# bystrogenomics/bystro-vcf

Measured on AMD Instinct MI355X. Metric: variants/sec, higher is better.
Workload: dtype u8; 1 GPU; BASELINE configs[2]: 1KG-Phase3 chr1-shaped, 2504 samples, biallelic SNPs; rows_per_block=311296, resident_blocks_per_gpu=8, n_samples=2504, input=resident in HBM, blocks_in_flight=3, flags=default (--allowFilter PASS,.), class maps on

## Files before the change

bystro-vcf_amd/__init__.py:

```python
import ctypes as C
import os

import numpy as np

try:
    import torch
except ImportError:
    torch = None

_HERE = os.path.dirname(os.path.abspath(__file__))
LIB_PATH = os.environ.get("BVCF_LIB") or os.path.join(_HERE, "libbvcf.so")

if not os.path.exists(LIB_PATH):
    raise ImportError(
        "bystro-vcf_amd: %s not built (run `python -c 'import __graft_entry__ as g; g.build()'` "
        "or `make -C bystro-vcf_amd/csrc`); there is no fallback path" % LIB_PATH)

lib = C.CDLL(LIB_PATH)

ABI_VERSION = 9
ABI_VERSION_SUBSET = 10
DEVICE_PAD = 64
NO_CMAP = 0xFFFFFFFF

OK, E_ARG, E_HIP, E_NODEV, E_BUSY, E_EMPTY, E_TOO_BIG, E_CAPACITY, E_NOMEM, E_FATAL = 0, -1, -2, -3, -4, -5, -6, -7, -8, -9
LINE_OK, LINE_FIELDS, LINE_FILTER, LINE_NOALLELE = 0, 1, 2, 3
SITE_NAMES = ["SNP", "INS", "DEL", "MNP", "MULTIALLELIC"]
ALT_BASE, ALT_INS, ALT_DEL = 0, 1, 2
CLS_NONE, CLS_HET, CLS_HOM, CLS_MISSING = 0, 1, 2, 3
SAMPLE_STATS_COLUMNS = ["sample", "het", "hom", "missing", "transitions", "transversions", "heterozygosity", "homozygosity",
                        "missingness", "trTv"]

BENCH_EXPORTS = ["bvcf_bench_device", "bvcf_bench_device_slots", "bvcf_bench_stream_kernel", "bvcf_bench_head_left"]

PLAN_EXPORTS = ["bvcf_plan_text_ranges", "bvcf_plan_bgzf_ranges", "bvcf_cut_text_range", "bvcf_find_bgzf_chain",
                "bvcf_plan_threads", "bvcf_plan_fd", "bvcf_head_fast_line"]

EXPORTS = [
    "bvcf_create", "bvcf_destroy", "bvcf_last_error", "bvcf_version", "bvcf_reserve", "bvcf_set_sample_names", "bvcf_set_row_format", "bvcf_alloc_pinned", "bvcf_alloc_pinned_near", "bvcf_warmup",
    "bvcf_free_pinned", "bvcf_submit", "bvcf_submit_device", "bvcf_submit_bgzf", "bvcf_collect", "bvcf_sample_stats", "bvcf_counters", "bvcf_sum_counters",
    "bvcf_allreduce_counters", "bvcf_device_count", "bvcf_device_pci_bus_id", "bvcf_path", "bvcf_config_defaults", "bvcf_string_header", "bvcf_format_tsv", "bvcf_run_buffer", "bvcf_run_fd", "bvcf_decompress_fd", "bvcf_bgzf_inflate_device", "bvcf_bgzf_deflate_device", "bvcf_free",
    "bvcf_arrow_open", "bvcf_arrow_append", "bvcf_arrow_close",
]


class Params(C.Structure):
    _fields_ = [
        ("abi_version", C.c_uint32), ("device", C.c_int32), ("n_header_fields", C.c_uint32),
        ("eol_chars", C.c_uint32), ("eol_byte", C.c_uint8), ("want_class_maps", C.c_uint8),
        ("want_dosage", C.c_uint8), ("want_name_lists", C.c_uint8), ("allow_filter", C.c_char_p), ("exclude_filter", C.c_char_p),
        ("max_batch_bytes", C.c_uint64), ("max_lines", C.c_uint32), ("max_alleles", C.c_uint32),
        ("cmap_bytes", C.c_uint64), ("n_slots", C.c_uint32), ("path", C.c_uint32),
        ("packed_sites", C.c_uint32), ("render_sites", C.c_uint32), ("want_sample_stats", C.c_uint32),
        ("min_gq", C.c_uint32), ("min_dp", C.c_uint32), ("sample_keep", C.POINTER(C.c_uint32)),
    ]


class Config(C.Structure):
    _fields_ = [
# ... 104 lines not shown
MODE_STREAM, MODE_TEXT_RANGES, MODE_BGZF_RANGES = 0, 1, 2
BGZF_SKIP_FIRST_LINE, BGZF_END_OF_STREAM = 1, 2
lib.bvcf_plan_text_ranges.argtypes = [C.c_uint64, C.c_uint64, C.c_uint64, C.c_uint64, C.POINTER(RangePlan)]
lib.bvcf_plan_bgzf_ranges.argtypes = [C.c_uint64, C.c_uint64, C.c_uint32, C.c_uint64, C.POINTER(RangePlan)]
lib.bvcf_cut_text_range.argtypes = [C.c_char_p, C.c_uint64, C.c_uint64, C.c_int, C.c_int, C.c_uint8, C.POINTER(TextCut)]
lib.bvcf_find_bgzf_chain.argtypes = [C.c_char_p, C.c_size_t, C.c_size_t]
lib.bvcf_find_bgzf_chain.restype = C.c_long
lib.bvcf_plan_threads.argtypes = [C.c_uint32, C.c_uint32, C.c_int, C.POINTER(ThreadBudget)]
lib.bvcf_plan_fd.argtypes = [C.c_int, C.c_int, C.c_uint32, C.c_uint64, C.c_int, C.POINTER(PlanBlock), C.c_size_t,
                             C.POINTER(C.c_size_t), C.POINTER(C.c_int), C.POINTER(RangePlan)]


def plan_fd(fd_in, n_workers, max_batch_bytes=0, device_inflate=1, fd_err=2, cap=1 << 16):
    out = (PlanBlock * cap)()
    n = C.c_size_t(0)
    mode = C.c_int(-1)
    plan = RangePlan()
    rc = lib.bvcf_plan_fd(fd_in, fd_err, n_workers, max_batch_bytes, device_inflate, out, cap, C.byref(n), C.byref(mode), C.byref(plan))
    assert n.value <= cap, "more blocks than room"
    return rc, mode.value, plan, [out[i] for i in range(n.value)]


HEAD_FAST_DECLINE, HEAD_FAST_PASS, HEAD_FAST_FILTER = 0, 1, 2
HAS_HEAD_BITS, NOT_REGULAR, DEFERRED = 0x80000000, 0x40000000, 0xFFFFFFFE


def head_fast_line(head, ls, len_flags, counts, cmap_off, tab_bits, line, n_header, allow="PASS,.", exclude=""):
    lib.bvcf_head_fast_line.argtypes = [C.c_char_p, C.c_uint32, C.c_uint32, C.c_uint32, C.POINTER(C.c_uint32), C.c_uint32,
                                        C.POINTER(C.c_uint32), C.c_uint32, C.c_uint32, C.c_char_p, C.c_char_p, C.c_void_p, C.c_void_p]
    L = np.zeros(1, dtype=LINE_DTYPE)
    A = np.zeros(1, dtype=ALLELE_DTYPE)
    v = lib.bvcf_head_fast_line(bytes(head), len(head), ls, len_flags, (C.c_uint32 * 5)(*counts), cmap_off,
                                (C.c_uint32 * 8)(*tab_bits), line, n_header, allow.encode(), exclude.encode(),
                                L.ctypes.data, A.ctypes.data)
    return v, (L[0] if v != HEAD_FAST_DECLINE else None), (A[0] if v == HEAD_FAST_PASS else None)


class BvcfError(RuntimeError):
    def __init__(self, rc, msg):
        super().__init__("bvcf error %d: %s" % (rc, msg))
        self.rc = rc


def make_config(cfg=None, device=0, max_batch_bytes=0, n_format_threads=0):
    cfg = cfg or {}
    c = Config()
    lib.bvcf_config_defaults(C.byref(c))
    keep = [cfg.get("emptyField", "!").encode(), cfg.get("fieldDelimiter", ";").encode(),
            cfg.get("allow", "PASS,.").encode(), cfg.get("exclude", "").encode()]
    c.empty_field, c.field_delimiter, c.allow_filter, c.exclude_filter = keep
    c.keep_id = int(cfg.get("keepId", False))
    c.keep_info = int(cfg.get("keepInfo", False))
    c.keep_pos = int(cfg.get("keepPos", False))
    c.normalize_header = int(cfg.get("normalizeHeader", True))
    c.device = device
    c.max_batch_bytes = max_batch_bytes
    c.n_format_threads = n_format_threads
    if cfg.get("sample"):
        keep.append(cfg["sample"].encode())
# ... 404 lines not shown
```

bystro-vcf_amd/csrc/bvcf_common.hip.h:

```cpp
#pragma once

#include <hip/hip_runtime.h>
#include <stdint.h>

#include "../../include/bvcf.h"

namespace bvcf_dev {


constexpr int kWave = 64;
constexpr int kWavesPerWg = 4;
constexpr int kWgThreads = kWave * kWavesPerWg;
constexpr uint32_t kChunk = 1024;
constexpr uint32_t kMaxProducerWaves = 32768;
constexpr uint32_t kScanGroup = 1024;

typedef uint32_t u32x4 __attribute__((ext_vector_type(4)));
typedef u32x4 u32x4_u __attribute__((aligned(1)));

struct FilterTable {
  uint32_t allow_nil, allow_n;
  uint32_t deny_nil, deny_n;
  uint16_t allow_off[32], allow_len[32];
  uint16_t deny_off[32], deny_len[32];
// ... 70 lines not shown
  uint32_t fused;
  uint32_t gen_stream;
  uint32_t wide;
  uint32_t win_bytes;
  uint32_t win_tabs_cap;
  uint32_t *win_tabs;
  uint32_t tile_bytes;
  uint32_t tile_quota;
  uint32_t n_tiles;
  StreamEntry *entries;
  uint32_t *line_len;
  uint32_t *line_cmap;
  uint16_t *head_bits;
  uint32_t *line_bits;
  uint32_t *finish_items;
  uint32_t *real_tasks;
  uint32_t *left_lines;
  uint32_t head_fast;
  uint32_t s1_fmode;
  uint32_t s1_fkey[4], s1_flen[4];
};
constexpr uint32_t kHasHeadBits = 0x80000000u;
constexpr uint32_t kNotRegular = 0x40000000u;


__device__ __forceinline__ int lane_id() { return threadIdx.x & (kWave - 1); }

__device__ __forceinline__ uint32_t wave_incl_scan(uint32_t v) {
  v += (uint32_t)__builtin_amdgcn_update_dpp(0, (int)v, 0x111, 0xF, 0xF, true);
  v += (uint32_t)__builtin_amdgcn_update_dpp(0, (int)v, 0x112, 0xF, 0xF, true);
  v += (uint32_t)__builtin_amdgcn_update_dpp(0, (int)v, 0x114, 0xF, 0xF, true);
  v += (uint32_t)__builtin_amdgcn_update_dpp(0, (int)v, 0x118, 0xF, 0xF, true);
  v += (uint32_t)__builtin_amdgcn_update_dpp(0, (int)v, 0x142, 0xA, 0xF, false);
  v += (uint32_t)__builtin_amdgcn_update_dpp(0, (int)v, 0x143, 0xC, 0xF, false);
  return v;
}

__device__ __forceinline__ uint32_t wave_incl_scan_max(uint32_t v) {
  v = max(v, (uint32_t)__builtin_amdgcn_update_dpp(0, (int)v, 0x111, 0xF, 0xF, true));
  v = max(v, (uint32_t)__builtin_amdgcn_update_dpp(0, (int)v, 0x112, 0xF, 0xF, true));
  v = max(v, (uint32_t)__builtin_amdgcn_update_dpp(0, (int)v, 0x114, 0xF, 0xF, true));
  v = max(v, (uint32_t)__builtin_amdgcn_update_dpp(0, (int)v, 0x118, 0xF, 0xF, true));
  v = max(v, (uint32_t)__builtin_amdgcn_update_dpp(0, (int)v, 0x142, 0xA, 0xF, false));
  v = max(v, (uint32_t)__builtin_amdgcn_update_dpp(0, (int)v, 0x143, 0xC, 0xF, false));
  return v;
}
// ... 82 lines not shown
```

bystro-vcf_amd/csrc/bvcf_core.hip:

```cpp
#include "bvcf_device.hip.h"
#include "../../include/bvcf_bench.h"
#include "../../include/bvcf_plan.h"
#include "bvcf_bgzf.h"
#include "bvcf_bgzf_out.h"

#include <dlfcn.h>
#include <rccl/rccl.h>
#include <stdio.h>
#include <stdlib.h>
#include <string.h>

#include <algorithm>
#include <mutex>
#include <string>
#include <thread>
#include <vector>

using namespace bvcf_dev;

namespace {

struct Slot {
  hipStream_t stream = nullptr;
  bool used_gen = false;
// ... 2042 lines not shown
  if (fill_filter(allow_filter, true, &ft.allow_nil, &ft.allow_n, ft.allow_off, ft.allow_len, ft.text, &used) ||
      fill_filter(exclude_filter, false, &ft.deny_nil, &ft.deny_n, ft.deny_off, ft.deny_len, ft.text, &used))
    return -1;
  HeadFastHostBytes hb;
  memset(&hb, 0, sizeof hb);
  memcpy(hb.b, head, std::min<size_t>(head_bytes, kHeadFastBytes + 16));
  StreamEntry en;
  en.ls = ls;
  en.len = len_flags;
  en.ac = counts[0];
  en.an = counts[1];
  en.n_het = counts[2];
  en.n_hom = counts[3];
  en.n_miss = counts[4];
  en.cmap_off = cmap_off;
  HeadFastHostOut out;
  memset(&out, 0, sizeof out);
  const int v = head_fast_eval(en, tab_bits, hb, line, n_header, &ft, out);
  if (v != kHeadFastDecline) memcpy(out_line, out.Lw, sizeof out.Lw);
  if (v == kHeadFastPass) memcpy(out_allele, out.Aw, sizeof out.Aw);
  return v;
}

int bvcf_counters(bvcf_ctx *c, uint64_t out[8]) {
  if (!c || !out) return BVCF_E_ARG;
  memcpy(out, c->totals, sizeof c->totals);
  return BVCF_OK;
}

int bvcf_sum_counters(bvcf_ctx *const *ctxs, int n, uint64_t out[8]) {
  if (!ctxs || n < 0 || !out) return BVCF_E_ARG;
  for (int k = 0; k < 8; k++) out[k] = 0;
  for (int i = 0; i < n; i++) {
    if (!ctxs[i]) return BVCF_E_ARG;
    for (int k = 0; k < 8; k++) out[k] += ctxs[i]->totals[k];
  }
  return BVCF_OK;
}

int bvcf_bgzf_inflate_device(int device, const uint8_t *comp, size_t n_comp, uint8_t *out, size_t cap, size_t *n_out) {
  if ((!comp && n_comp) || !n_out || (!out && cap)) return BVCF_E_ARG;
  *n_out = 0;
  int n_dev = 0;
  if (hipGetDeviceCount(&n_dev) != hipSuccess || device < 0 || device >= n_dev) return BVCF_E_NODEV;
  std::vector<bvcf_bgzf::Block> blocks;
  const long used = bvcf_bgzf::scan(comp, n_comp, &blocks);
// ... 259 lines not shown
```

bystro-vcf_amd/csrc/bvcf_headfast.hip.h:

```cpp
#pragma once

#include <stddef.h>

#include "bvcf_common.hip.h"

namespace bvcf_dev {

constexpr uint32_t kHeadFastBytes = 64;
constexpr uint32_t kHeadFastFilter = 16;
constexpr uint32_t kHfNoTask = 0xFFFFFFFFu;
constexpr uint32_t kHfDeferred = 0xFFFFFFFEu;

enum { kHeadFastDecline = 0, kHeadFastPass = 1, kHeadFastFilterFail = 2 };

static_assert(sizeof(bvcf_line) == 64 && sizeof(bvcf_allele) == 64, "records are written as sixteen words");
static_assert(offsetof(bvcf_line, fend) == 8 && offsetof(bvcf_line, rec_first) == 44 && offsetof(bvcf_line, n_rec) == 48 &&
                  offsetof(bvcf_line, n_fields) == 52 && offsetof(bvcf_line, gt_task) == 56 && offsetof(bvcf_line, status) == 60 &&
                  offsetof(bvcf_line, site_type) == 61,
              "bvcf_line words");
static_assert(offsetof(bvcf_allele, line) == 8 && offsetof(bvcf_allele, alt_idx) == 12 && offsetof(bvcf_allele, alt_off) == 16 &&
                  offsetof(bvcf_allele, alt_len) == 20 && offsetof(bvcf_allele, ac) == 24 && offsetof(bvcf_allele, n_miss) == 40 &&
                  offsetof(bvcf_allele, cmap_off) == 44 && offsetof(bvcf_allele, ref) == 48 && offsetof(bvcf_allele, alt_base) == 49 &&
                  offsetof(bvcf_allele, kind) == 50 && offsetof(bvcf_allele, site_type) == 51 && offsetof(bvcf_allele, trtv) == 52 &&
                  offsetof(bvcf_allele, flags) == 53 && offsetof(bvcf_allele, gt_task) == 56,
              "bvcf_allele words");

__host__ __device__ __forceinline__ bool hf_is_actg(uint32_t c) {
  const uint32_t d = c - 'A';
  return d < 20u && ((0x80045u >> (d & 31u)) & 1u);
}

__host__ __device__ __forceinline__ uint32_t hf_trtv(uint32_t ref, uint32_t alt) {
  const uint32_t x = ((ref ^ alt) >> 1) & 3u;
  return (hf_is_actg(ref) && hf_is_actg(alt)) ? (x == 3u ? 1u : 2u) : 0u;
}

__host__ __device__ __forceinline__ uint32_t hf_next_bit(unsigned long long x[4]) {
  uint32_t pos = 256u;
  bool done = false;
#pragma unroll
  for (uint32_t q = 0; q < 4; q++) {
    const bool take = !done && x[q] != 0ull;
    if (take) {
      pos = 64u * q + (uint32_t)__builtin_ctzll(x[q]);
      x[q] &= x[q] - 1ull;
    }
    done = done || take;
  }
  return pos;
}

__host__ __device__ __forceinline__ uint32_t hf_byte16(const uint32_t v[4], uint32_t k) {
  const uint32_t w = k < 8u ? (k < 4u ? v[0] : v[1]) : (k < 12u ? v[2] : v[3]);
  return (w >> (8u * (k & 3u))) & 0xFFu;
}

__host__ __device__ inline bool hf_filter_in(const uint32_t f[4], uint32_t n, const uint16_t *off, const uint16_t *len, uint32_t cnt,
                                             const uint8_t *text) {
  bool hit = false;
  for (uint32_t i = 0; i < cnt; i++) {
    const uint32_t kl = len[i];
    if (kl > kHeadFastFilter) continue;
    bool eq = kl == n;
    for (uint32_t k = 0; k < kl; k++) eq = eq && hf_byte16(f, k) == text[off[i] + k];
    hit = hit || eq;
  }
  return hit;
}

template <class H, class Out>
__host__ __device__ inline int head_fast_eval(const StreamEntry &en, const uint32_t bits[8], const H &head, uint32_t g, uint32_t n_header,
                                              const FilterTable *ft, Out &out) {
  if (!(en.len & kHasHeadBits) || (en.len & kNotRegular) || en.n_miss == kHfDeferred || n_header <= 9u) return kHeadFastDecline;
  const uint32_t ls = en.ls, len = en.len & ~(kHasHeadBits | kNotRegular), sh = ls & 3u;
  unsigned long long x[4];
#pragma unroll
  for (uint32_t q = 0; q < 4; q++) x[q] = ((unsigned long long)bits[2 * q + 1] << 32) | bits[2 * q];
  uint32_t t[9];
#pragma unroll
  for (uint32_t i = 0; i < 9; i++) t[i] = hf_next_bit(x) - sh;
  if (t[8] + sh >= 256u) return kHeadFastDecline;
  if (t[6] >= kHeadFastBytes || t[8] >= len) return kHeadFastDecline;
  if (t[3] - t[2] != 2u || t[4] - t[3] != 2u) return kHeadFastDecline;
  const uint32_t f_off = t[5] + 1u, f_len = t[6] - f_off;
  if (f_len > kHeadFastFilter) return kHeadFastDecline;
  const uint32_t ref = head.byte(t[2] + 1u), alt = head.byte(t[3] + 1u);
  uint32_t fv[4];
  head.bytes16(f_off, fv);
  if (!hf_is_actg(alt) || alt == ref) return kHeadFastDecline;
  bool pass = true;
  if (!ft->allow_nil && !hf_filter_in(fv, f_len, ft->allow_off, ft->allow_len, ft->allow_n, ft->text))
    pass = false;
  else if (!ft->deny_nil && hf_filter_in(fv, f_len, ft->deny_off, ft->deny_len, ft->deny_n, ft->text))
    pass = false;
  uint32_t Lw[16];
  Lw[0] = ls;
  Lw[1] = len;
#pragma unroll
  for (uint32_t i = 0; i < 9; i++) Lw[2 + i] = t[i];
  Lw[11] = 0;
  Lw[12] = pass ? 1u : 0u;
  Lw[13] = pass ? n_header : 0u;
  Lw[14] = g;
  Lw[15] = pass ? (uint32_t)BVCF_LINE_OK | ((uint32_t)BVCF_SITE_SNP << 8) : (uint32_t)BVCF_LINE_FILTER;
  out.line(Lw);
  if (!pass) return kHeadFastFilterFail;
  uint32_t Aw[16];
  const uint32_t cm = en.cmap_off;
  const bool sparse = cm != BVCF_NO_CMAP && (cm & 1u);
  Aw[0] = Aw[1] = 0;
  Aw[2] = g;
  Aw[3] = 0;
  Aw[4] = 0;
  Aw[5] = 1;
  Aw[6] = en.ac;
  Aw[7] = en.an;
  Aw[8] = en.n_het;
  Aw[9] = en.n_hom;
  Aw[10] = en.n_miss;
  Aw[11] = cm != BVCF_NO_CMAP ? cm & ~15u : cm;
  Aw[12] = ref | (alt << 8) | ((uint32_t)BVCF_ALT_BASE << 16) | ((uint32_t)BVCF_SITE_SNP << 24);
  Aw[13] = hf_trtv(ref, alt) | ((BVCF_ALLELE_POS_TEXT | (sparse ? BVCF_ALLELE_CMAP_SPARSE : 0u)) << 8);
  Aw[14] = g;
  Aw[15] = 0;
  out.allele(Aw);
  return kHeadFastPass;
}

struct HeadFastHostBytes {
  uint8_t b[kHeadFastBytes + 16];
  __host__ __device__ uint32_t byte(uint32_t rel) const { return b[rel]; }
  __host__ __device__ void bytes16(uint32_t rel, uint32_t out[4]) const {
#pragma unroll
    for (uint32_t q = 0; q < 4; q++)
      out[q] = (uint32_t)b[rel + 4 * q] | ((uint32_t)b[rel + 4 * q + 1] << 8) | ((uint32_t)b[rel + 4 * q + 2] << 16) |
               ((uint32_t)b[rel + 4 * q + 3] << 24);
  }
};

struct HeadFastHostOut {
  uint32_t Lw[16], Aw[16];
  void line(const uint32_t w[16]) {
    for (int i = 0; i < 16; i++) Lw[i] = w[i];
  }
  void allele(const uint32_t w[16]) {
    for (int i = 0; i < 16; i++) Aw[i] = w[i];
  }
};

}
```

bystro-vcf_amd/csrc/bvcf_stream.hip.h:

```cpp
#pragma once

#include <type_traits>

#include "bvcf_common.hip.h"
#include "bvcf_gtscan.hip.h"
#include "bvcf_headfast.hip.h"

namespace bvcf_dev {


constexpr uint32_t kNone = 0xFFFFFFFFu;
constexpr uint32_t kDeferred = 0xFFFFFFFEu;
static_assert(kDeferred == kHfDeferred, "head_fast_eval's copy");

__device__ inline uint32_t find_eol(const KernelArgs &a, uint32_t from, uint32_t limit) {
  const int lane = lane_id();
  const uint32_t last_off = (a.cap - 16u) & ~3u;
  for (uint32_t base = from & ~3u; base < limit; base += 4u * kChunk) {
    u32x4 v[4];
#pragma unroll
    for (int q = 0; q < 4; q++) v[q] = ld_stream(a.buf + min(base + q * kChunk + 16u * lane, last_off));
#pragma unroll
    for (int q = 0; q < 4; q++) {
      const uint32_t off = base + q * kChunk + 16u * lane;
// ... 26 lines not shown
  const unsigned long long be = __ballot(me != 0);
  uint32_t eol_here = kNone;
  if (be) {
    const int src = __ffsll((long long)be) - 1;
    eol_here = lane_value(off + __ffs(me) - 1, src);
    mt &= bits_until(eol_here, off);
  }
  uint32_t tot;
  const uint32_t cnt = __popc(mt);
  const uint32_t prefix = wave_excl_scan(cnt, &tot);
  if (*found_io + tot >= need) {
    const uint32_t target = need - 1 - *found_io;
    const bool mine = prefix <= target && target < prefix + cnt;
    const unsigned long long bm = __ballot(mine);
    const int src = __ffsll((long long)bm) - 1;
    const uint32_t pos = mine ? off + nth_bit(mt, target - prefix) : 0u;
    return lane_value(pos, src);
  }
  *found_io += tot;
  *eolp = eol_here;
  return kNone;
}

__device__ __forceinline__ uint32_t head_window16(const KernelArgs &a, u32x4 v, uint32_t start, uint32_t *mt_out) {
  const int lane = lane_id();
  const uint32_t need = 9;
  const uint32_t base = start & ~3u;
  if (lane == 0) v.x &= 0xFFFFFFFFu << (8u * (start & 3u));
  const uint32_t off = base + 16u * lane;
  uint32_t valid = bits_until(a.nbytes, off);
  if (lane >= 16) valid = 0;
  const uint32_t e4 = a.eol_byte * 0x01010101u;
  const uint32_t eol_any = (zero_bytes(v.x ^ e4) | zero_bytes(v.y ^ e4) | zero_bytes(v.z ^ e4) | zero_bytes(v.w ^ e4));
  if (__ballot(eol_any != 0 && lane < 16)) return kNone;
  const uint32_t mt = eq_mask16(v, '\t') & valid;
  *mt_out = mt;
  const uint32_t cnt = __popc(mt);
  uint32_t x = cnt;
  x += (uint32_t)__builtin_amdgcn_update_dpp(0, (int)x, 0x111, 0xF, 0xF, true);
  x += (uint32_t)__builtin_amdgcn_update_dpp(0, (int)x, 0x112, 0xF, 0xF, true);
  x += (uint32_t)__builtin_amdgcn_update_dpp(0, (int)x, 0x114, 0xF, 0xF, true);
  x += (uint32_t)__builtin_amdgcn_update_dpp(0, (int)x, 0x118, 0xF, 0xF, true);
  const uint32_t prefix = x - cnt;
  const bool mine = lane < 16 && prefix < need && need <= x;
  const unsigned long long bm = __ballot(mine);
  if (!bm) return kNone;
  const int src = __ffsll((long long)bm) - 1;
  const uint32_t pos = mine ? off + nth_bit(mt, need - 1 - prefix) : 0u;
  return lane_value(pos, src);
}

constexpr int kPipeChunks = 10;

#ifdef BVCF_EXP_TIMES
__device__ unsigned long long g_wave_t[2][32768];
__device__ unsigned long long g_phase_t[8][32768];
__device__ unsigned int g_wave_hw[2][32768];
#if BVCF_EXP_TIMES + 0 == 2
#define STAMP(k)
#else
#define STAMP(k)                                                   \
  {                                                                \
    const unsigned long long now_ = __builtin_readcyclecounter();  \
    ph_[k] += now_ - last_;                                        \
    last_ = now_;                                                  \
  }
#endif
#else
#define STAMP(k)
#endif
__global__ __launch_bounds__(kWgThreads) void k_stream(KernelArgs a) {
#ifdef BVCF_EXP_TIMES
// ... 33 lines not shown
  uint32_t p = kNone;
  if (tile_lo < tile_hi) {
    p = 0;
    if (r0 > 0) {
      const uint32_t q = find_eol(a, r0 - 1, r1);
      p = q == kNone ? kNone : q + 1;
    }
  }

  const uint32_t lines_bound = (uint32_t)(((unsigned long long)per_wave * T) / (4ull * ns + 8ull)) + 2u;
  const uint32_t slots_per_wave = lines_bound + lines_bound / 4u;
  cm_next = wave * slots_per_wave;
  cm_end = cm_next + slots_per_wave;
  if (maps && wave == 0 && lane == 0)
    a.counters->cmap_maps = min(n_waves, a.n_tiles) * slots_per_wave;
  auto map_slot = [&]() -> uint32_t {
    if (!maps) return BVCF_NO_CMAP;
    if (cm_next >= cm_end) {
      if (lane == 0) a.counters->pad[0] = 1;
      return BVCF_NO_CMAP;
    }
    return cmap_of(a, cm_next, true);
  };
  auto commit = [&](uint32_t ls, uint32_t cend, const GtStats &st, bool deferred, uint32_t cm_off, bool bits_ok = false,
                    uint32_t bits = 0u, uint32_t n_slots = 1u) {
    while (ls >= (tile + 1) * T) {
      if (lane == 0) a.census[tile] = n_local;
      n_listed += n_local;
      tile++;
      n_local = 0;
    }
    if (n_local >= a.tile_quota) {
      if (lane == 0) a.counters->pad[0] = 1;
      return;
    }
    if (lane == 0) {
      StreamEntry en;
      en.ls = ls;
      en.len = (cend - ls) | (bits_ok ? kHasHeadBits : 0u);
      en.ac = st.ac;
      en.an = st.an;
      en.n_het = st.n_het;
      en.n_hom = st.n_hom;
      en.n_miss = deferred ? kDeferred : st.n_miss;
      en.cmap_off = cm_off;
      a.entries[(size_t)tile * a.tile_quota + n_local] = en;
    }
    if (bits_ok && lane < 16) a.head_bits[((size_t)tile * a.tile_quota + n_local) * 16u + (uint32_t)lane] = (uint16_t)bits;
    n_local++;
    if (maps && !deferred) cm_next += n_slots;
  };
  const uint32_t amask = (ns & 255u) ? 3u : 0u;
  const uint32_t cap_off = (a.cap - 16u) & ~3u;
  auto chunk_off = [&](uint32_t s_begin, uint32_t c) -> uint32_t {
    return min((s_begin & ~amask) + c * kChunk + 16u * lane, cap_off);
  };
  auto chunk_at = [&](uint32_t s_begin, uint32_t c) -> u32x4 { return ld_stream(a.buf + chunk_off(s_begin, c)); };
  auto finish_stats = [&](const FastAcc &acc, GtStats *st) {
    wave_sum3(acc.het, acc.hom, acc.miss, ns, &st->n_het, &st->n_hom, &st->n_miss);
    st->ac = st->n_het + 2u * st->n_hom;
    st->an = 2u * (ns - st->n_miss);
  };

  while (p != kNone && p < r1) {
// ... 2 lines not shown
      tab9 = head_window(a, load16(a.buf, base + 16u * lane, a.cap), base, kWave, &found, &eolp);
      if (tab9 != kNone || eolp != kNone) break;
    }
    if (tab9 == kNone) {
      if (eolp == kNone) break;
      seen++;
      p = eolp + 1;
      continue;
    }
    uint32_t s_begin = tab9 + 1;
    GtStats st = {0, 0, 0, 0, 0};
    const unsigned long long pred = (unsigned long long)s_begin + 4ull * ns - 1ull;
    uint32_t cend = kNone;

    if (pred + a.eol_chars <= nb && pipelined) {
      auto run_pipeline = [&](auto loads_tag) {
        constexpr int kLoads = decltype(loads_tag)::value;
        constexpr uint32_t nc = kLoads;
        uint32_t pA = p, sA = s_begin, peA = (uint32_t)pred;
        u32x4 va[kPipeChunks];
        u32x4 hv = {0u, 0u, 0u, 0u};
        uint32_t mtA = 0, mtB = 0;
        bool bitsA = false;
        auto head_at = [&](uint32_t start) -> u32x4 {
          return *reinterpret_cast<const u32x4_u *>(a.buf + min((start & ~3u) + 16u * (lane & 15), cap_off));
        };
        bool hv_ok = peA + 1u < r1;
        hv = head_at(hv_ok ? peA + 1u : sA);
#pragma unroll
        for (int g = 0; g < kPipeChunks; g++) va[g] = g < kLoads ? chunk_at(sA, g) : u32x4{0u, 0u, 0u, 0u};
        for (;;) {
          STAMP(0);
          uint32_t sB = 0, peB = 0;
          bool b_ok = false;
          if (hv_ok) {
            const uint32_t t9 = head_window16(a, hv, peA + 1u, &mtB);
            if (t9 != kNone) {
              sB = t9 + 1;
              const unsigned long long pb = (unsigned long long)sB + 4ull * ns - 1ull;
              if (pb + 1ull <= nb) {
                peB = (uint32_t)pb;
                b_ok = true;
              }
            }
          }
          const bool hvc_ok = b_ok && peB + 1u < r1;
          hv = head_at(hvc_ok ? peB + 1u : sA);
          STAMP(1);
          const uint32_t cmA = bcast0(map_slot());
          uint8_t *cm = cmA != BVCF_NO_CMAP ? a.cmap + cmA : nullptr;
#ifdef BVCF_EXP_NO_SPARSE
          const bool sparse_ok = false;
#else
          const bool sparse_ok = cm != nullptr && a.cmap_stride >= 4u * kSparseWords;
#endif
          FastAcc acc = {0, 0, 0, 0, sparse_ok ? 0u : kDenseMode};
          if (cm && !sparse_ok) zero_stage(stage, nc);
          const uint32_t rA = sA & amask;
          const uint32_t w0 = __builtin_amdgcn_alignbyte(__builtin_amdgcn_readfirstlane(va[0].y),
                                                         __builtin_amdgcn_readfirstlane(va[0].x), rA);
// ... 16 lines not shown
          uint32_t enc = 0, n_slots = 1;
          const uint32_t raw_slots = (kRawAreaBytes + a.cmap_stride - 1u) / a.cmap_stride;
          auto raw_area = [&]() -> uint8_t * {
            const uint32_t reserve = (r1 - min(r1, peA)) / (4u * ns + 8u) + 2u;
            if (cm_next + 1u + raw_slots + reserve > cm_end || cmap_of(a, cm_next + raw_slots, true) == BVCF_NO_CMAP) return nullptr;
            return cm + a.cmap_stride;
          };
          if (sparse_ok && acc.n_sp < kDenseMode) {
            enc = finish_list(sparse, acc, cm, min(kListAlleles, a.cmap_stride / (4u * kSparseWords)), stage, nc, a.cmap_stride,
                              acc.n_sp > BVCF_CMAP_SPARSE_MAX ? raw_area() : nullptr);
          } else if (sparse_ok && acc.n_oth == 0u) {
            enc = 1u << 1;
          } else if (sparse_ok && acc.n_oth < kDenseMode) {
            enc = finish_dense(sparse, acc.n_oth, raw_area());
          }
          if (enc == kRawEnc) n_slots += raw_slots;
          if (__any(acc.bad != 0)) {
            s_begin = sA;
            p = pA;
            break;
          }
          finish_stats(acc, &st);
          seen++;
          commit(pA, peA, st, false, cmA == BVCF_NO_CMAP ? cmA : cmA | enc, bitsA, mtA, n_slots);
          p = peA + 1u;
          if (!b_ok) {
            s_begin = kNone;
            break;
          }
          pA = peA + 1u;
          sA = sB;
          peA = peB;
          hv_ok = hvc_ok;
          mtA = mtB;
#ifdef BVCF_EXP_NO_HEAD_BITS
          bitsA = false;
#else
          bitsA = true;
#endif
          STAMP(4);
        }
      };
      switch (n_chunks) {
        case 1: run_pipeline(std::integral_constant<int, 1>{}); break;
        case 2: run_pipeline(std::integral_constant<int, 2>{}); break;
        case 3: run_pipeline(std::integral_constant<int, 3>{}); break;
        case 4: run_pipeline(std::integral_constant<int, 4>{}); break;
        case 5: run_pipeline(std::integral_constant<int, 5>{}); break;
        case 6: run_pipeline(std::integral_constant<int, 6>{}); break;
        case 7: run_pipeline(std::integral_constant<int, 7>{}); break;
        case 8: run_pipeline(std::integral_constant<int, 8>{}); break;
        case 9: run_pipeline(std::integral_constant<int, 9>{}); break;
        default: run_pipeline(std::integral_constant<int, 10>{}); break;
      }
      static_assert(kPipeChunks == 10, "the dispatch above covers 1..10 chunks");
      if (s_begin == kNone) continue;
    } else if (pred + a.eol_chars <= nb) {
      const uint32_t pe = (uint32_t)pred;
      bool term = true;
      if (a.eol_chars == 2) term = a.buf[pe + 1] == a.eol_byte && a.buf[pe] != a.eol_byte;
      if (term) {
// ... 26 lines not shown
    }
  }
  for (; tile < tile_hi; tile++) {
    if (lane == 0) a.census[tile] = n_local;
    n_listed += n_local;
    n_local = 0;
  }
  if (lane == 0) a.run_lines[wave] = n_listed;
  if (lane == 0 && seen) atomicAdd(&a.counters->lines_seen, seen);
  if (lane == 0 && n_other) atomicAdd(&a.counters->n_other_shape, n_other);
#ifdef BVCF_EXP_TIMES
  if (lane == 0) {
    g_wave_t[1][wave] = wall_clock64();
    for (int k = 0; k < 8; k++) g_phase_t[k][wave] = ph_[k];
  }
#endif
}

}
#include "bvcf_streamgen.hip.h"
namespace bvcf_dev {

struct HeadFastDeviceBytes {
  const uint8_t *p;
  uint32_t room;
  __device__ __forceinline__ uint32_t byte(uint32_t rel) const { return rel < room ? p[rel] : 0u; }
  __device__ __forceinline__ void bytes16(uint32_t rel, uint32_t out[4]) const {
    const u32x4 v = load16(p, rel, room);
    out[0] = v.x;
    out[1] = v.y;
    out[2] = v.z;
    out[3] = v.w;
  }
};

struct HeadFastDeviceOut {
  u32x4 *lp, *ap;
  __device__ __forceinline__ static void put(u32x4 *d, const uint32_t w[16]) {
#pragma unroll
    for (uint32_t q = 0; q < 4; q++) d[q] = u32x4{w[4 * q], w[4 * q + 1], w[4 * q + 2], w[4 * q + 3]};
  }
  __device__ __forceinline__ void line(const uint32_t w[16]) { put(lp, w); }
  __device__ __forceinline__ void allele(const uint32_t w[16]) { put(ap, w); }
};

__global__ __launch_bounds__(kWgThreads) void k_order(KernelArgs a) {
  __shared__ uint32_t s_part[2][kWavesPerWg];
  __shared__ uint32_t s_first[kWgThreads + 1];
  const int lane = lane_id();
  const uint32_t w = threadIdx.x >> 6;
  if (a.n_tiles == 0) {
    if (blockIdx.x == 0 && threadIdx.x == 0) a.counters->n_lines = 0;
    return;
  }
  const uint32_t pw = a.prod_waves;
  const uint32_t q_tiles = a.n_tiles / pw, r_tiles = a.n_tiles % pw;
  auto run_first = [&](uint32_t wv) -> uint32_t { return wv * q_tiles + min(wv, r_tiles); };
  const uint32_t per_wg = (pw + gridDim.x - 1u) / gridDim.x;
  const uint32_t w_lo = min(blockIdx.x * per_wg, pw), w_hi = min(w_lo + per_wg, pw);
  const uint32_t t_lo = run_first(w_lo), t_hi = run_first(w_hi);
  uint32_t sum = 0;
  {
    const uint32_t n4 = w_lo / 4u;
    const u32x4 *c4 = reinterpret_cast<const u32x4 *>(a.run_lines);
    for (uint32_t i = threadIdx.x; i < n4; i += kWgThreads) {
// ... 25 lines not shown
    for (uint32_t i = 0; i < kWavesPerWg; i++) {
      if (i < w) wbase += s_part[1][i];
      total += s_part[1][i];
    }
    s_first[threadIdx.x] = wbase + pre;
    if (threadIdx.x == 0) s_first[kWgThreads] = total;
    __syncthreads();
    const uint32_t n_round = s_first[kWgThreads];
    for (uint32_t j0 = 0; j0 < n_round; j0 += kWgThreads) {
      const uint32_t j = j0 + threadIdx.x;
      const uint32_t g = base + j;
      const bool live = j < n_round && g < a.max_lines;
      bool left = false;
      if (live) {
        uint32_t lo = 0;
#pragma unroll
        for (uint32_t s = kWgThreads / 2u; s >= 1u; s >>= 1)
          if (s_first[lo + s] <= j) lo += s;
        const uint32_t tl = lo, k = j - s_first[lo];
        const size_t ei = (size_t)(c0 + tl) * a.tile_quota + k;
        const u32x4 *ep = reinterpret_cast<const u32x4 *>(a.entries + ei);
        const u32x4 *bp = reinterpret_cast<const u32x4 *>(a.head_bits + ei * 16u);
        const u32x4 e0 = ep[0], e1 = ep[1];
        const u32x4 b0 = bp[0], b1 = bp[1];
        StreamEntry en;
        en.ls = e0.x;
        en.len = e0.y;
        en.ac = e0.z;
        en.an = e0.w;
        en.n_het = e1.x;
        en.n_hom = e1.y;
        en.n_miss = e1.z;
        en.cmap_off = e1.w;
        if (g < a.max_tasks) {
          GtResult r;
          r.ac = en.ac;
          r.an = en.an;
          r.n_het = en.n_het;
          r.n_hom = en.n_hom;
          r.n_miss = en.n_miss;
          r.n_fields = en.n_miss == kDeferred ? kDeferred : a.n_header - 9u;
          r.regular = (en.n_miss == kDeferred || (en.len & kNotRegular)) ? 0u : 1u;
          r.pad = 0;
          a.results[g] = r;
        }
        int verdict = kHeadFastDecline;
        if (a.head_fast && (en.len & kHasHeadBits) && g < a.max_alleles && g < a.max_tasks) {
          const uint32_t bits[8] = {b0.x, b0.y, b0.z, b0.w, b1.x, b1.y, b1.z, b1.w};
          const HeadFastDeviceBytes head = {a.buf + en.ls, a.cap - min(a.cap, en.ls)};
          HeadFastDeviceOut out = {reinterpret_cast<u32x4 *>(a.lines + g), reinterpret_cast<u32x4 *>(a.alleles + g)};
          verdict = head_fast_eval(en, bits, head, g, a.n_header, a.filters, out);
          if (verdict == kHeadFastFilterFail) a.alleles[g].gt_task = kHfNoTask;
        }
        if (verdict == kHeadFastDecline) {
          left = true;
          a.line_off[g] = en.ls;
          a.line_len[g] = en.len & ~kNotRegular;
          a.line_cmap[g] = en.cmap_off;
          if (en.len & kHasHeadBits) {
            u32x4 *dst = reinterpret_cast<u32x4 *>(a.line_bits + (size_t)g * 8u);
            dst[0] = bp[0];
            dst[1] = bp[1];
          }
        }
      }
      const unsigned long long lm = __ballot(left);
      if (lm) {
        uint32_t at = 0;
        if (lane == 0) at = atomicAdd(&a.counters->n_left, (uint32_t)__popcll(lm));
        at = bcast0(at) + __builtin_amdgcn_mbcnt_hi((uint32_t)(lm >> 32), __builtin_amdgcn_mbcnt_lo((uint32_t)lm, 0u));
        if (left) a.left_lines[at] = g;
      }
    }
    base += s_first[kWgThreads];
  }
  if (t_hi == a.n_tiles && threadIdx.x == 0) a.counters->n_lines = base;
}


}
// ... 1 lines not shown
```

include/bvcf_plan.h:

```cpp
#ifndef BVCF_PLAN_H
#define BVCF_PLAN_H

#include <stddef.h>
#include <stdint.h>

#include "bvcf.h"

#ifdef __cplusplus
extern "C" {
#endif

typedef struct {
  uint64_t data_off;
  uint64_t range_bytes;
  uint64_t spare_bytes;
  uint64_t n_ranges;
} bvcf_range_plan;

int bvcf_plan_text_ranges(uint64_t file_size, uint64_t data_off, uint64_t max_batch_bytes, uint64_t first_line_bytes,
                          bvcf_range_plan *out);
int bvcf_plan_bgzf_ranges(uint64_t file_size, uint64_t data_off, uint32_t n_workers, uint64_t max_batch_bytes,
                          bvcf_range_plan *out);

enum {
// ... 21 lines not shown
int bvcf_plan_threads(uint32_t cpus, uint32_t n_workers, int mode, bvcf_thread_budget *out);

typedef struct {
  uint32_t worker;
  uint32_t piece;
  uint64_t range;
  uint64_t file_off;
  uint64_t nbytes;
  uint64_t own;
  uint32_t first_off;
  uint8_t bgzf;
  uint8_t bgzf_flags;
  uint8_t last_piece;
  uint8_t reserved;
} bvcf_plan_block;

int bvcf_plan_fd(int fd_in, int fd_err, uint32_t n_workers, uint64_t max_batch_bytes, int device_inflate,
                 bvcf_plan_block *out, size_t cap, size_t *n_out, int *mode_out, bvcf_range_plan *plan_out);

int bvcf_head_fast_line(const uint8_t *head, uint32_t head_bytes, uint32_t ls, uint32_t len_flags, const uint32_t counts[5],
                        uint32_t cmap_off, const uint32_t tab_bits[8], uint32_t line, uint32_t n_header, const char *allow_filter,
                        const char *exclude_filter, bvcf_line *out_line, bvcf_allele *out_allele);

#ifdef __cplusplus
}
#endif
#endif
```

Baseline: 515.5 million variants/s.

## Encode tab positions in stream entries to skip head-bit buffer for plain lines

```diff
diff --git a/bystro-vcf_amd/__init__.py b/bystro-vcf_amd/__init__.py
--- a/bystro-vcf_amd/__init__.py
+++ b/bystro-vcf_amd/__init__.py
@@ -34,7 +34,7 @@
 BENCH_EXPORTS = ["bvcf_bench_device", "bvcf_bench_device_slots", "bvcf_bench_stream_kernel", "bvcf_bench_head_left"]
 
 PLAN_EXPORTS = ["bvcf_plan_text_ranges", "bvcf_plan_bgzf_ranges", "bvcf_cut_text_range", "bvcf_find_bgzf_chain",
-                "bvcf_plan_threads", "bvcf_plan_fd", "bvcf_head_fast_line"]
+                "bvcf_plan_threads", "bvcf_plan_fd", "bvcf_head_fast_line", "bvcf_head_fast_text_line"]
 
 EXPORTS = [
     "bvcf_create", "bvcf_destroy", "bvcf_last_error", "bvcf_version", "bvcf_reserve", "bvcf_set_sample_names", "bvcf_set_row_format", "bvcf_alloc_pinned", "bvcf_alloc_pinned_near", "bvcf_warmup",
@@ -185,7 +185,7 @@
 
 
 HEAD_FAST_DECLINE, HEAD_FAST_PASS, HEAD_FAST_FILTER = 0, 1, 2
-HAS_HEAD_BITS, NOT_REGULAR, DEFERRED = 0x80000000, 0x40000000, 0xFFFFFFFE
+HAS_HEAD_BITS, NOT_REGULAR, PLAIN_HEAD, DEFERRED = 0x80000000, 0x40000000, 0x20000000, 0xFFFFFFFE
 
 
 def head_fast_line(head, ls, len_flags, counts, cmap_off, tab_bits, line, n_header, allow="PASS,.", exclude=""):
@@ -198,6 +198,19 @@
                                 L.ctypes.data, A.ctypes.data)
     return v, (L[0] if v != HEAD_FAST_DECLINE else None), (A[0] if v == HEAD_FAST_PASS else None)
 
+
+
+def head_fast_text_line(head, ls, length, counts, cmap_off, tab7, tab8, line, n_header, allow="PASS,.", exclude=""):
+    lib.bvcf_head_fast_text_line.argtypes = [C.c_char_p, C.c_uint32, C.c_uint32, C.c_uint32, C.POINTER(C.c_uint32), C.c_uint32,
+                                             C.c_uint32, C.c_uint32, C.c_uint32, C.c_uint32, C.c_char_p, C.c_char_p, C.c_void_p,
+                                             C.c_void_p]
+    L = np.zeros(1, dtype=LINE_DTYPE)
+    A = np.zeros(1, dtype=ALLELE_DTYPE)
+    v = lib.bvcf_head_fast_text_line(bytes(head), len(head), ls, length, (C.c_uint32 * 5)(*counts), cmap_off, tab7, tab8, line,
+                                     n_header, allow.encode(), exclude.encode(), L.ctypes.data, A.ctypes.data)
+    if v < 0:
+        raise ValueError("bvcf_head_fast_text_line: bad arguments")
+    return v, (L[0] if v != HEAD_FAST_DECLINE else None), (A[0] if v == HEAD_FAST_PASS else None)
 
 class BvcfError(RuntimeError):
     def __init__(self, rc, msg):
diff --git a/bystro-vcf_amd/csrc/bvcf_common.hip.h b/bystro-vcf_amd/csrc/bvcf_common.hip.h
--- a/bystro-vcf_amd/csrc/bvcf_common.hip.h
+++ b/bystro-vcf_amd/csrc/bvcf_common.hip.h
@@ -116,6 +116,9 @@
 };
 constexpr uint32_t kHasHeadBits = 0x80000000u;
 constexpr uint32_t kNotRegular = 0x40000000u;
+constexpr uint32_t kPlainHead = 0x20000000u;
+__host__ __device__ __forceinline__ uint32_t plain_pack(uint32_t tab7, uint32_t tab8) { return tab7 | (tab8 << 8); }
+__host__ __device__ __forceinline__ uint32_t plain_an(uint32_t n_samples, uint32_t n_miss) { return 2u * (n_samples - n_miss); }
 
 
 __device__ __forceinline__ int lane_id() { return threadIdx.x & (kWave - 1); }
diff --git a/bystro-vcf_amd/csrc/bvcf_core.hip b/bystro-vcf_amd/csrc/bvcf_core.hip
--- a/bystro-vcf_amd/csrc/bvcf_core.hip
+++ b/bystro-vcf_amd/csrc/bvcf_core.hip
@@ -2088,6 +2088,38 @@
   return v;
 }
 
+int bvcf_head_fast_text_line(const uint8_t *head, uint32_t head_bytes, uint32_t ls, uint32_t len, const uint32_t counts[5],
+                             uint32_t cmap_off, uint32_t tab7, uint32_t tab8, uint32_t line, uint32_t n_header, const char *allow_filter,
+                             const char *exclude_filter, bvcf_line *out_line, bvcf_allele *out_allele) {
+  if (!head || !counts || !out_line || !out_allele || tab7 >= 256u || tab8 >= 256u || (len & (kHasHeadBits | kNotRegular | kPlainHead)))
+    return -1;
+  if (n_header > 9u && counts[4] != kHfDeferred && counts[1] != plain_an(n_header - 9u, counts[4])) return -1;
+  FilterTable ft;
+  memset(&ft, 0, sizeof ft);
+  uint32_t used = 0;
+  if (fill_filter(allow_filter, true, &ft.allow_nil, &ft.allow_n, ft.allow_off, ft.allow_len, ft.text, &used) ||
+      fill_filter(exclude_filter, false, &ft.deny_nil, &ft.deny_n, ft.deny_off, ft.deny_len, ft.text, &used))
+    return -1;
+  HeadFastHostBytes hb;
+  memset(&hb, 0, sizeof hb);
+  memcpy(hb.b, head, std::min<size_t>(head_bytes, kHeadFastBytes + 16));
+  StreamEntry en;
+  en.ls = ls;
+  en.len = len | kPlainHead;
+  en.ac = counts[0];
+  en.an = plain_pack(tab7, tab8);
+  en.n_het = counts[2];
+  en.n_hom = counts[3];
+  en.n_miss = counts[4];
+  en.cmap_off = cmap_off;
+  HeadFastHostOut out;
+  memset(&out, 0, sizeof out);
+  const int v = head_fast_eval(en, nullptr, hb, line, n_header, &ft, out);
+  if (v != kHeadFastDecline) memcpy(out_line, out.Lw, sizeof out.Lw);
+  if (v == kHeadFastPass) memcpy(out_allele, out.Aw, sizeof out.Aw);
+  return v;
+}
+
 int bvcf_counters(bvcf_ctx *c, uint64_t out[8]) {
   if (!c || !out) return BVCF_E_ARG;
   memcpy(out, c->totals, sizeof c->totals);
diff --git a/bystro-vcf_amd/csrc/bvcf_headfast.hip.h b/bystro-vcf_amd/csrc/bvcf_headfast.hip.h
--- a/bystro-vcf_amd/csrc/bvcf_headfast.hip.h
+++ b/bystro-vcf_amd/csrc/bvcf_headfast.hip.h
@@ -35,21 +35,6 @@
   return (hf_is_actg(ref) && hf_is_actg(alt)) ? (x == 3u ? 1u : 2u) : 0u;
 }
 
-__host__ __device__ __forceinline__ uint32_t hf_next_bit(unsigned long long x[4]) {
-  uint32_t pos = 256u;
-  bool done = false;
-#pragma unroll
-  for (uint32_t q = 0; q < 4; q++) {
-    const bool take = !done && x[q] != 0ull;
-    if (take) {
-      pos = 64u * q + (uint32_t)__builtin_ctzll(x[q]);
-      x[q] &= x[q] - 1ull;
-    }
-    done = done || take;
-  }
-  return pos;
-}
-
 __host__ __device__ __forceinline__ uint32_t hf_byte16(const uint32_t v[4], uint32_t k) {
   const uint32_t w = k < 8u ? (k < 4u ? v[0] : v[1]) : (k < 12u ? v[2] : v[3]);
   return (w >> (8u * (k & 3u))) & 0xFFu;
@@ -68,42 +53,87 @@
   return hit;
 }
 
+__host__ __device__ __forceinline__ uint32_t hf_tab_mask4(uint32_t w) {
+  const uint32_t x = w ^ 0x09090909u;
+  const uint32_t z = ~(((x & 0x7F7F7F7Fu) + 0x7F7F7F7Fu) | x | 0x7F7F7F7Fu) >> 7;
+  return (z | (z >> 7) | (z >> 14) | (z >> 21)) & 0xFu;
+}
+
 template <class H, class Out>
 __host__ __device__ inline int head_fast_eval(const StreamEntry &en, const uint32_t bits[8], const H &head, uint32_t g, uint32_t n_header,
                                               const FilterTable *ft, Out &out) {
-  if (!(en.len & kHasHeadBits) || (en.len & kNotRegular) || en.n_miss == kHfDeferred || n_header <= 9u) return kHeadFastDecline;
-  const uint32_t ls = en.ls, len = en.len & ~(kHasHeadBits | kNotRegular), sh = ls & 3u;
-  unsigned long long x[4];
+  const uint32_t len_flags = en.len;
+  if (!(len_flags & (kHasHeadBits | kPlainHead)) || (len_flags & kNotRegular) || en.n_miss == kHfDeferred || n_header <= 9u)
+    return kHeadFastDecline;
+  const uint32_t ls = en.ls, len = len_flags & ~(kHasHeadBits | kNotRegular | kPlainHead), sh = ls & 3u;
+  uint32_t t[9];
+  {
+    unsigned long long x = 0ull;
 #pragma unroll
-  for (uint32_t q = 0; q < 4; q++) x[q] = ((unsigned long long)bits[2 * q + 1] << 32) | bits[2 * q];
-  uint32_t t[9];
+    for (uint32_t q = 0; q < kHeadFastBytes / 16u; q++) {
+      uint32_t v[4];
+      head.bytes16(16u * q, v);
 #pragma unroll
-  for (uint32_t i = 0; i < 9; i++) t[i] = hf_next_bit(x) - sh;
-  if (t[8] + sh >= 256u) return kHeadFastDecline;
-  if (t[6] >= kHeadFastBytes || t[8] >= len) return kHeadFastDecline;
+      for (uint32_t k = 0; k < 4; k++) x |= (unsigned long long)hf_tab_mask4(v[k]) << (16u * q + 4u * k);
+    }
+#pragma unroll
+    for (uint32_t i = 0; i < 7; i++) {
+      t[i] = x ? (uint32_t)__builtin_ctzll(x) : kHeadFastBytes;
+      x &= x - 1ull;
+    }
+  }
+  if (t[6] >= kHeadFastBytes) return kHeadFastDecline;
   if (t[3] - t[2] != 2u || t[4] - t[3] != 2u) return kHeadFastDecline;
+  uint32_t w7 = 256u, w8 = 256u, an;
+  if (len_flags & kPlainHead) {
+    w7 = en.an & 0xFFu;
+    w8 = (en.an >> 8) & 0xFFu;
+    an = plain_an(n_header - 9u, en.n_miss);
+  } else {
+    an = en.an;
+    uint32_t seen = 0;
+#pragma nounroll
+    for (uint32_t q = 0; q < 8u && seen < 9u; q++) {
+      uint32_t m = bits[q];
+      while (m && seen < 9u) {
+        const uint32_t pos = 32u * q + (uint32_t)__builtin_ctz(m);
+        m &= m - 1u;
+        if (seen == 7u) w7 = pos;
+        if (seen == 8u) w8 = pos;
+        seen++;
+      }
+    }
+    if (w8 >= 256u) return kHeadFastDecline;
+  }
+  t[7] = w7 - sh;
+  t[8] = w8 - sh;
+  if (t[7] <= t[6] || t[8] <= t[7] || t[8] >= len) return kHeadFastDecline;
   const uint32_t f_off = t[5] + 1u, f_len = t[6] - f_off;
   if (f_len > kHeadFastFilter) return kHeadFastDecline;
   const uint32_t ref = head.byte(t[2] + 1u), alt = head.byte(t[3] + 1u);
+  if (!hf_is_actg(alt) || alt == ref) return kHeadFastDecline;
+  {
+    uint32_t Fw[12];
+    Fw[0] = ls;
+    Fw[1] = len;
+#pragma unroll
+    for (uint32_t i = 0; i < 9; i++) Fw[2 + i] = t[i];
+    Fw[11] = 0;
+    out.line_fields(Fw);
+  }
   uint32_t fv[4];
   head.bytes16(f_off, fv);
-  if (!hf_is_actg(alt) || alt == ref) return kHeadFastDecline;
   bool pass = true;
   if (!ft->allow_nil && !hf_filter_in(fv, f_len, ft->allow_off, ft->allow_len, ft->allow_n, ft->text))
     pass = false;
   else if (!ft->deny_nil && hf_filter_in(fv, f_len, ft->deny_off, ft->deny_len, ft->deny_n, ft->text))
     pass = false;
-  uint32_t Lw[16];
-  Lw[0] = ls;
-  Lw[1] = len;
-#pragma unroll
-  for (uint32_t i = 0; i < 9; i++) Lw[2 + i] = t[i];
-  Lw[11] = 0;
-  Lw[12] = pass ? 1u : 0u;
-  Lw[13] = pass ? n_header : 0u;
-  Lw[14] = g;
-  Lw[15] = pass ? (uint32_t)BVCF_LINE_OK | ((uint32_t)BVCF_SITE_SNP << 8) : (uint32_t)BVCF_LINE_FILTER;
-  out.line(Lw);
+  uint32_t Vw[4];
+  Vw[0] = pass ? 1u : 0u;
+  Vw[1] = pass ? n_header : 0u;
+  Vw[2] = g;
+  Vw[3] = pass ? (uint32_t)BVCF_LINE_OK | ((uint32_t)BVCF_SITE_SNP << 8) : (uint32_t)BVCF_LINE_FILTER;
+  out.line_verdict(Vw);
   if (!pass) return kHeadFastFilterFail;
   uint32_t Aw[16];
   const uint32_t cm = en.cmap_off;
@@ -114,7 +144,7 @@
   Aw[4] = 0;
   Aw[5] = 1;
   Aw[6] = en.ac;
-  Aw[7] = en.an;
+  Aw[7] = an;
   Aw[8] = en.n_het;
   Aw[9] = en.n_hom;
   Aw[10] = en.n_miss;
@@ -140,8 +170,11 @@
 
 struct HeadFastHostOut {
   uint32_t Lw[16], Aw[16];
-  void line(const uint32_t w[16]) {
-    for (int i = 0; i < 16; i++) Lw[i] = w[i];
+  void line_fields(const uint32_t w[12]) {
+    for (int i = 0; i < 12; i++) Lw[i] = w[i];
+  }
+  void line_verdict(const uint32_t w[4]) {
+    for (int i = 0; i < 4; i++) Lw[12 + i] = w[i];
   }
   void allele(const uint32_t w[16]) {
     for (int i = 0; i < 16; i++) Aw[i] = w[i];
diff --git a/bystro-vcf_amd/csrc/bvcf_stream.hip.h b/bystro-vcf_amd/csrc/bvcf_stream.hip.h
--- a/bystro-vcf_amd/csrc/bvcf_stream.hip.h
+++ b/bystro-vcf_amd/csrc/bvcf_stream.hip.h
@@ -72,7 +72,7 @@
   return kNone;
 }
 
-__device__ __forceinline__ uint32_t head_window16(const KernelArgs &a, u32x4 v, uint32_t start, uint32_t *mt_out) {
+__device__ __forceinline__ uint32_t head_window16(const KernelArgs &a, u32x4 v, uint32_t start, uint32_t *mt_out, int *src_out) {
   const int lane = lane_id();
   const uint32_t need = 9;
   const uint32_t base = start & ~3u;
@@ -96,8 +96,25 @@
   const unsigned long long bm = __ballot(mine);
   if (!bm) return kNone;
   const int src = __ffsll((long long)bm) - 1;
+  *src_out = src;
   const uint32_t pos = mine ? off + nth_bit(mt, need - 1 - prefix) : 0u;
   return lane_value(pos, src);
+}
+
+__device__ __forceinline__ bool plain_shaped(uint32_t mt, uint32_t t9, int src, uint32_t base, uint32_t *t78) {
+  const unsigned long long m = (unsigned long long)(lane_value(mt, 0) | (lane_value(mt, 1) << 16)) |
+                               ((unsigned long long)(lane_value(mt, 2) | (lane_value(mt, 3) << 16)) << 32);
+  unsigned long long m2 = m & (m - 1ull);
+  m2 &= m2 - 1ull;
+  const bool head_ok = __popcll(m) >= 7 && ((m2 >> (__builtin_ctzll(m2 | (1ull << 63)) & 63)) & 0x1Full) == 0x15ull;
+  const uint32_t lo = src > 0 ? lane_value(mt, src > 0 ? src - 1 : 0) : 0u;
+  const uint32_t w = lo | (lane_value(mt, src) << 16);
+  const uint32_t w_base = 16u * (uint32_t)src - 16u;
+  const uint32_t b8 = (t9 - base) - w_base;
+  const uint32_t below = w & ((1u << (b8 & 31u)) - 1u);
+  const uint32_t b7 = 31u - (uint32_t)__builtin_clz(below | 1u);
+  *t78 = plain_pack(w_base + b7, t9 - base);
+  return head_ok && below != 0u;
 }
 
 constexpr int kPipeChunks = 10;
@@ -177,8 +194,10 @@
     }
     return cmap_of(a, cm_next, true);
   };
+  const bool head_fast = a.head_fast != 0;
   auto commit = [&](uint32_t ls, uint32_t cend, const GtStats &st, bool deferred, uint32_t cm_off, bool bits_ok = false,
-                    uint32_t bits = 0u, uint32_t n_slots = 1u) {
+                    uint32_t bits = 0u, uint32_t n_slots = 1u,
+                    bool plain = false, uint32_t t78 = 0u) {
     while (ls >= (tile + 1) * T) {
       if (lane == 0) a.census[tile] = n_local;
       n_listed += n_local;
@@ -192,9 +211,9 @@
     if (lane == 0) {
       StreamEntry en;
       en.ls = ls;
-      en.len = (cend - ls) | (bits_ok ? kHasHeadBits : 0u);
+      en.len = (cend - ls) | (bits_ok ? kHasHeadBits : 0u) | (plain ? kPlainHead : 0u);
       en.ac = st.ac;
-      en.an = st.an;
+      en.an = plain ? t78 : st.an;
       en.n_het = st.n_het;
       en.n_hom = st.n_hom;
       en.n_miss = deferred ? kDeferred : st.n_miss;
@@ -243,6 +262,8 @@
         u32x4 hv = {0u, 0u, 0u, 0u};
         uint32_t mtA = 0, mtB = 0;
         bool bitsA = false;
+        bool plainA = false, plainB = false;
+        uint32_t t78A = 0, t78B = 0;
         auto head_at = [&](uint32_t start) -> u32x4 {
           return *reinterpret_cast<const u32x4_u *>(a.buf + min((start & ~3u) + 16u * (lane & 15), cap_off));
         };
@@ -255,8 +276,11 @@
           uint32_t sB = 0, peB = 0;
           bool b_ok = false;
           if (hv_ok) {
-            const uint32_t t9 = head_window16(a, hv, peA + 1u, &mtB);
+            int srcB = 0;
+            const uint32_t t9 = head_window16(a, hv, peA + 1u, &mtB, &srcB);
+            plainB = false;
             if (t9 != kNone) {
+              if (head_fast) plainB = plain_shaped(mtB, t9, srcB, (peA + 1u) & ~3u, &t78B);
               sB = t9 + 1;
               const unsigned long long pb = (unsigned long long)sB + 4ull * ns - 1ull;
               if (pb + 1ull <= nb) {
@@ -319,7 +343,7 @@
           }
           finish_stats(acc, &st);
           seen++;
-          commit(pA, peA, st, false, cmA == BVCF_NO_CMAP ? cmA : cmA | enc, bitsA, mtA, n_slots);
+          commit(pA, peA, st, false, cmA == BVCF_NO_CMAP ? cmA : cmA | enc, bitsA, mtA, n_slots, plainA, t78A);
           p = peA + 1u;
           if (!b_ok) {
             s_begin = kNone;
@@ -333,7 +357,9 @@
 #ifdef BVCF_EXP_NO_HEAD_BITS
           bitsA = false;
 #else
-          bitsA = true;
+          bitsA = !plainB;
+          plainA = plainB;
+          t78A = t78B;
 #endif
           STAMP(4);
         }
@@ -406,11 +432,12 @@
 namespace bvcf_dev {
 
 struct HeadFastDeviceBytes {
-  const uint8_t *p;
-  uint32_t room;
-  __device__ __forceinline__ uint32_t byte(uint32_t rel) const { return rel < room ? p[rel] : 0u; }
+  const uint8_t *buf;
+  uint32_t ls;
+  uint32_t cap;
+  __device__ __forceinline__ uint32_t byte(uint32_t rel) const { return ls + rel < cap ? buf[ls + rel] : 0u; }
   __device__ __forceinline__ void bytes16(uint32_t rel, uint32_t out[4]) const {
-    const u32x4 v = load16(p, rel, room);
+    const u32x4 v = load16(buf, ls + rel, cap);
     out[0] = v.x;
     out[1] = v.y;
     out[2] = v.z;
@@ -424,7 +451,11 @@
 #pragma unroll
     for (uint32_t q = 0; q < 4; q++) d[q] = u32x4{w[4 * q], w[4 * q + 1], w[4 * q + 2], w[4 * q + 3]};
   }
-  __device__ __forceinline__ void line(const uint32_t w[16]) { put(lp, w); }
+  __device__ __forceinline__ void line_fields(const uint32_t w[12]) {
+#pragma unroll
+    for (uint32_t q = 0; q < 3; q++) lp[q] = u32x4{w[4 * q], w[4 * q + 1], w[4 * q + 2], w[4 * q + 3]};
+  }
+  __device__ __forceinline__ void line_verdict(const uint32_t w[4]) { lp[3] = u32x4{w[0], w[1], w[2], w[3]}; }
   __device__ __forceinline__ void allele(const uint32_t w[16]) { put(ap, w); }
 };
 
@@ -496,7 +527,6 @@
         const u32x4 *ep = reinterpret_cast<const u32x4 *>(a.entries + ei);
         const u32x4 *bp = reinterpret_cast<const u32x4 *>(a.head_bits + ei * 16u);
         const u32x4 e0 = ep[0], e1 = ep[1];
-        const u32x4 b0 = bp[0], b1 = bp[1];
         StreamEntry en;
         en.ls = e0.x;
         en.len = e0.y;
@@ -506,10 +536,18 @@
         en.n_hom = e1.y;
         en.n_miss = e1.z;
         en.cmap_off = e1.w;
-        if (g < a.max_tasks) {
+        int verdict = kHeadFastDecline;
+        if (a.head_fast && (en.len & (kHasHeadBits | kPlainHead)) && g < a.max_alleles && g < a.max_tasks) {
+          const HeadFastDeviceBytes head = {a.buf, en.ls, a.cap};
+          HeadFastDeviceOut out = {reinterpret_cast<u32x4 *>(a.lines + g), reinterpret_cast<u32x4 *>(a.alleles + g)};
+          verdict = head_fast_eval(en, reinterpret_cast<const uint32_t *>(bp), head, g, a.n_header, a.filters, out);
+          if (verdict == kHeadFastFilterFail) a.alleles[g].gt_task = kHfNoTask;
+        }
+        left = verdict == kHeadFastDecline;
+        if (g < a.max_tasks && (left || a.dosage != nullptr)) {
           GtResult r;
           r.ac = en.ac;
-          r.an = en.an;
+          r.an = (en.len & kPlainHead) ? plain_an(a.n_header - 9u, en.n_miss) : en.an;
           r.n_het = en.n_het;
           r.n_hom = en.n_hom;
           r.n_miss = en.n_miss;
@@ -518,18 +556,9 @@
           r.pad = 0;
           a.results[g] = r;
         }
-        int verdict = kHeadFastDecline;
-        if (a.head_fast && (en.len & kHasHeadBits) && g < a.max_alleles && g < a.max_tasks) {
-          const uint32_t bits[8] = {b0.x, b0.y, b0.z, b0.w, b1.x, b1.y, b1.z, b1.w};
-          const HeadFastDeviceBytes head = {a.buf + en.ls, a.cap - min(a.cap, en.ls)};
-          HeadFastDeviceOut out = {reinterpret_cast<u32x4 *>(a.lines + g), reinterpret_cast<u32x4 *>(a.alleles + g)};
-          verdict = head_fast_eval(en, bits, head, g, a.n_header, a.filters, out);
-          if (verdict == kHeadFastFilterFail) a.alleles[g].gt_task = kHfNoTask;
-        }
-        if (verdict == kHeadFastDecline) {
-          left = true;
+        if (left) {
           a.line_off[g] = en.ls;
-          a.line_len[g] = en.len & ~kNotRegular;
+          a.line_len[g] = en.len & ~(kNotRegular | kPlainHead);
           a.line_cmap[g] = en.cmap_off;
           if (en.len & kHasHeadBits) {
             u32x4 *dst = reinterpret_cast<u32x4 *>(a.line_bits + (size_t)g * 8u);
diff --git a/include/bvcf_plan.h b/include/bvcf_plan.h
--- a/include/bvcf_plan.h
+++ b/include/bvcf_plan.h
@@ -67,6 +67,10 @@
                         uint32_t cmap_off, const uint32_t tab_bits[8], uint32_t line, uint32_t n_header, const char *allow_filter,
                         const char *exclude_filter, bvcf_line *out_line, bvcf_allele *out_allele);
 
+int bvcf_head_fast_text_line(const uint8_t *head, uint32_t head_bytes, uint32_t ls, uint32_t len, const uint32_t counts[5],
+                             uint32_t cmap_off, uint32_t tab7, uint32_t tab8, uint32_t line, uint32_t n_header, const char *allow_filter,
+                             const char *exclude_filter, bvcf_line *out_line, bvcf_allele *out_allele);
+
 #ifdef __cplusplus
 }
 #endif
```

Result: no change. 511.5 million variants/s, median of 2 (-0.8%).
